# nelpy/ghost

Hardware: AMD Instinct MI355X
Metric: Msamples/s CWT (128ch x 1e6 samp x 100 scales); % HBM roofline; 1/2/4/8 GPU (higher is better)
Workload: dtype f32

## Files before the change

ghost_amd/csrc/api.cpp:

```cpp
#include <hip/hip_runtime.h>

#include <algorithm>
#include <cmath>
#include <cstdio>
#include <cstdlib>
#include <cstring>
#include <exception>
#include <map>
#include <new>
#include <string>
#include <vector>

#include "../../include/ghostcwt.h"
#include "../../include/ghostcwt_debug.h"
#include <memory>

#include "errors.h"
#include "host_out.h"
#include "interp.h"
#include "kernels.h"
#include "morse_exact.h"
#include "morlet_exact.h"
#include "options.h"
#include "planner.h"

using namespace gcwt;

namespace {

thread_local std::string g_err;


int set_err(int code, const std::string& msg) {
  g_err = msg;
  return code;
}

int hip_err(hipError_t e, const char* what) {
  g_err = std::string(what) + ": " + hipGetErrorString(e);
  return e == hipErrorOutOfMemory ? GCWT_ERR_NOMEM : GCWT_ERR_HIP;
}

#define HIP_TRY(call)                                  \
  do {                                                 \
    hipError_t e_ = (call);                            \
    if (e_ != hipSuccess) return hip_err(e_, #call);   \
  } while (0)

struct EpochDev {
  SynthItemDev* items = nullptr;
  int n_items = 0;
  SynthLevelDev* levels = nullptr;
  Synth7Item* items7 = nullptr;
  Synth7Level* levels7 = nullptr;
  int n_items7 = 0;
  Synth7Item* items7w = nullptr;
  int n_items7w = 0;
  Synth7Item* items7n = nullptr;
  int n_items7n = 0;
  SynthiItem* items_i = nullptr;
  SynthiLevel* levels_i = nullptr;
  int n_items_i = 0;
  SynthpItem* items_p[2] = {nullptr, nullptr};
  SynthpLevel* levels_p = nullptr;
  int n_items_p[2] = {0, 0};
  PredLevel* pred_levels = nullptr;
};

constexpr int64_t kFullbandCacheBytes = (int64_t)16 << 30;

enum Stage { ST_MEAN = 0, ST_FWD, ST_DECIM, ST_BLOCK, ST_SYNTH, ST_DIRECT, ST_FULLBAND, ST_INTERP, ST_BLOCKCONV, ST_COUNT };

}

struct gcwt_plan {
  HostPlan hp;
  bool uploaded = false;
  int profiling = 0;
  int synth_cols = 32;
  int synth7_narrow_r = 2;
  bool fuse_blocks = true;
  int synth_kernel = 7;
  bool prune_inputs = true;
  bool fast_fft = true;
  int drop_stores = 0;
  bool clock_probe = false;
  bool use_synth16 = false;
  int device = -1;
  hipStream_t stream = nullptr;
  hipStream_t aux[2] = {nullptr, nullptr};
  bool level_streams = true;
  bool use_synthp = false;
  bool use_graphs = true;
  bool fullband4 = true;
  int fullband_group = 0;
  int64_t fullband_cache_cap = 0;
  bool hfull_cache_full = false;
  int synth7_order = 0;
  int synthp_help = -1;
  int synthp_lgnb = -1;
  int interp_lgnb = -1;
  int interp_grid = -1;
  bool last_fold = false;
  bool fold_mean = true;
  bool synth_streams = false;
  hipStream_t cur = nullptr;
  bool high_precision = true;
  double2* d_y = nullptr;
  int64_t y_stride = 0;
  double2* d_tw64 = nullptr;
  float2* d_x = nullptr;
  float2* d_xr = nullptr;
  float2* d_xb = nullptr;
  float2* d_bank = nullptr;
  float* d_gain = nullptr;
  float* d_gain_lv = nullptr;
  float2* d_half_tw = nullptr;
  float2* d_psi = nullptr;
  float2* d_psi_tail = nullptr;
  float2* d_psi_lit = nullptr;
  unsigned long long* d_probe = nullptr;
  double* d_amps = nullptr;
  float2* d_xs = nullptr;
  int64_t xs_stride = 0;
  float2* d_z = nullptr;
  int64_t z_half = 0;
  int z_sets = 1;
  float2* d_hfull = nullptr;
  std::map<std::pair<int, int>, float2*> hfull_cache;
  int64_t hfull_cache_bytes = 0;
  float2* d_tw4096 = nullptr;
  float2* d_tw256 = nullptr;
  float2* d_level_tw = nullptr;
  double* d_sums = nullptr;
  int32_t* d_scale_list = nullptr;
  int n_listed = 0;
  int32_t* d_scale_aux = nullptr;
  float* d_interp_coef = nullptr;
  BankScale* d_bank_sc = nullptr;
  DirectScale* d_direct_sc = nullptr;
  float2* d_bc_h = nullptr;
  int32_t* d_bc_rows = nullptr;
  float2* d_bc_x = nullptr;
  float2* d_bc_tw = nullptr;
  std::vector<EpochDev> ep_dev;
  int64_t max_direct_len = 0;
  float* d_in = nullptr;
  size_t d_in_bytes = 0;
  void* d_out = nullptr;
  size_t d_out_bytes = 0;
  HostOut host_out;
  std::vector<hipEvent_t> ev_pool;
  size_t ev_used = 0;
  struct Span { int stage; hipEvent_t a, b; };
  std::vector<Span> spans;
  gcwt_timings last{};
  bool have_timings = false;
  bool have_means = false;
  bool detect = false;
  float* d_hist = nullptr;
  float* d_bands = nullptr;
  float* d_pred = nullptr;
  hipStream_t det_stream = nullptr;
  int32_t* d_scale_level = nullptr;
  int32_t* d_scale_length = nullptr;
  std::vector<float> last_pred;
  float* h_pred = nullptr;
  float last_worst = 0.f;
  int last_rerouted = 0;
  float auto_threshold = 1.5e-6f;
  float kappa_eps = 1.6e-7f;
  float oob_tol = 2.5e-8f;
  int last_batch_slots = 0;
  int last_batch = 0, last_rows = 0;
  double last_pt = 0;
  gcwt_plan* sub_plan[2] = {nullptr, nullptr};
  bool is_sub_plan = false;
  const unsigned char* run_mask = nullptr;
  unsigned char* d_run_mask = nullptr;
  struct GraphKey {
    const void* x = nullptr; const void* out = nullptr;
    int64_t r0 = 0, r1 = 0, row_len = 0; bool reuse = false;
    bool operator==(const GraphKey& o) const {
      return x == o.x && out == o.out && r0 == o.r0 && r1 == o.r1 && row_len == o.row_len && reuse == o.reuse;
    }
  };
  GraphKey graph_key, graph_seen;
  hipGraphExec_t graph_exec = nullptr;
// ... 122 lines not shown
int gcwt_device_pci_bus_id(int device, char* buf, size_t buflen) {
  if (!buf || buflen < 16) return set_err(GCWT_ERR_INVALID, "buffer of at least 16 bytes needed");
  HIP_TRY(hipDeviceGetPCIBusId(buf, (int)buflen, device));
  return GCWT_OK;
}

int gcwt_set_device(int device) {
  int n = 0;
  if (hipGetDeviceCount(&n) != hipSuccess || n == 0) {
    (void)hipGetLastError();
    return set_err(GCWT_ERR_NO_DEVICE, "no HIP device: libghostcwt needs an AMD GPU (gfx950); there is no CPU path");
  }
  if (device < 0 || device >= n) return set_err(GCWT_ERR_NO_DEVICE, "no such device (gcwt_device_count tells how many there are)");
  HIP_TRY(hipSetDevice(device));
  return GCWT_OK;
}
int gcwt_current_device(int* device) {
  if (!device) return set_err(GCWT_ERR_INVALID, "NULL argument");
  HIP_TRY(hipGetDevice(device));
  return GCWT_OK;
}

int gcwt_device_memory(size_t* free_bytes, size_t* total_bytes) {
  if (!free_bytes || !total_bytes) return set_err(GCWT_ERR_INVALID, "NULL argument");
  HIP_TRY(hipMemGetInfo(free_bytes, total_bytes));
  return GCWT_OK;
}
int gcwt_device_malloc(void** ptr, size_t bytes) { HIP_TRY(hipMalloc(ptr, bytes ? bytes : 1)); return GCWT_OK; }
int gcwt_device_free(void* ptr) { HIP_TRY(hipFree(ptr)); return GCWT_OK; }
int gcwt_memcpy_h2d(void* dst, const void* src, size_t bytes) {
  HIP_TRY(hipMemcpy(dst, src, bytes, hipMemcpyHostToDevice)); return GCWT_OK;
}
int gcwt_memcpy_d2h(void* dst, const void* src, size_t bytes) {
  HIP_TRY(hipMemcpy(dst, src, bytes, hipMemcpyDeviceToHost)); return GCWT_OK;
}
int gcwt_device_memset(void* dst, int value, size_t bytes) {
  HIP_TRY(hipMemset(dst, value, bytes)); return GCWT_OK;
}
int gcwt_device_synchronize(void) { HIP_TRY(hipDeviceSynchronize()); return GCWT_OK; }
int gcwt_host_alloc(void** ptr, size_t bytes) {
  if (!ptr) return set_err(GCWT_ERR_INVALID, "NULL argument");
  HIP_TRY(hipHostMalloc(ptr, bytes ? bytes : 1, hipHostMallocDefault));
  return GCWT_OK;
}
int gcwt_host_free(void* ptr) { HIP_TRY(hipHostFree(ptr)); return GCWT_OK; }
int gcwt_rows_to_host(const float* d_src, int64_t src_pitch, int64_t n_rows, int64_t row_elems, void* dst,
                      int64_t dst_pitch, int flags) {
  return guarded([&] {
    if (!d_src || !dst) return set_err(GCWT_ERR_INVALID, "NULL argument");
    if (n_rows < 0 || row_elems < 0 || src_pitch < row_elems || dst_pitch < row_elems)
      return set_err(GCWT_ERR_INVALID, "bad rectangle (rows, elements per row, pitches)");
    if (!(flags & GCWT_HOST_PINNED) && dst_pitch != row_elems)
      return set_err(GCWT_ERR_INVALID, "a destination that is not page-locked takes dense rows (dst_pitch = row_elems)");
    HIP_TRY(rows_to_host(d_src, src_pitch, n_rows, row_elems, dst, dst_pitch, (flags & GCWT_OUT_F64) != 0,
                         (flags & GCWT_HOST_PINNED) != 0));
    return (int)GCWT_OK;
  });
}

static int gcwt_plan_create_impl(gcwt_plan** out, const gcwt_params* params) {
  if (!out || !params) return set_err(GCWT_ERR_INVALID, "NULL argument");
  *out = nullptr;
  std::unique_ptr<gcwt_plan> owner(new (std::nothrow) gcwt_plan());
  gcwt_plan* p = owner.get();
  if (!p) return set_err(GCWT_ERR_NOMEM, "out of host memory");
  std::string err;
  int rc = build_host_plan(*params, &p->hp, &err);
  if (rc != GCWT_OK) return set_err(rc, err);
  p->hp.prm.freqs_hz = p->hp.freqs.data();
  p->hp.prm.epoch_bounds = p->hp.bounds.data();
  p->hp.prm.n_epochs = (int32_t)(p->hp.bounds.size() / 2);
  p->device = params->device;
  p->high_precision = p->hp.high_precision;
  p->use_synth16 = option_or("synth16", 0) == 1;
  p->synth_cols = option_or("synth_cols", 32) == 16 ? 16 : 32;
  p->synth7_narrow_r = (int)option_or("synth7_narrow_r", 2);
  p->fuse_blocks = option_or("fuse_blocks", 1) != 0;
  p->prune_inputs = option_or("prune_inputs", 1) != 0;
  p->fast_fft = option_or("slow_fft", 0) == 0;
  p->level_streams = option_or("level_streams", 1) != 0;
  if (option_is_set("interp_grid")) p->interp_grid = option_or("interp_grid", 0) != 0;
  p->synth_streams = option_or("synth_streams", 0) != 0;
  p->fold_mean = option_or("fold_mean", 1) != 0;
  p->interp_lgnb = (int)option_or("interp_lgnb", -1);
  p->use_synthp = kMeasureBuild && option_or("synthp", 0) != 0;
  p->synthp_lgnb = (int)option_or("synthp_lgnb", -1);
  p->synthp_help = (int)option_or("synthp_help", -1);
  p->use_graphs = option_or("graphs", 1) != 0;
  p->synth7_order = (int)option_or("synth7_order", 0);
  p->auto_threshold = 1e-9f * (float)option_or("auto_threshold_ppb", 1500);
  p->kappa_eps = 1e-9f * (float)option_or("auto_kappa_ppb", 160);
  p->oob_tol = 1e-12f * (float)option_or("auto_oob_ppt", 25000);
  p->fullband_group = (int)option_or("fullband_group", 0);
  p->fullband4 = option_or("fullband4", 1) != 0;
  p->synth_kernel = kMeasureBuild && option_or("synth_kernel", 7) == 8 ? 8 : 7;
  p->drop_stores = kMeasureBuild && option_is_set("synth_drop_stores") ? (int)std::max<long long>(1, option_or("synth_drop_stores", 1)) : 0;
  p->clock_probe = kMeasureBuild && option_is_set("clock_probe");
  for (const auto& s : p->hp.scales)
    if (s.method == GCWT_SCALE_DIRECT) p->max_direct_len = std::max(p->max_direct_len, s.length);
  *out = owner.release();
  return GCWT_OK;
}

void gcwt_plan_destroy(gcwt_plan* plan) {
  if (!plan) return;
  if (plan->uploaded || plan->stream) {
    if (plan->device >= 0) (void)hipSetDevice(plan->device);
    free_dev(plan);
  }
  delete plan;
}

int gcwt_plan_get_info(const gcwt_plan* plan, gcwt_plan_info* info) {
  if (!plan || !info) return set_err(GCWT_ERR_INVALID, "NULL argument");
  const HostPlan& hp = plan->hp;
  info->abi_version = GCWT_ABI_VERSION;
  info->n_levels = (int32_t)hp.levels.size();
  info->n_direct = hp.n_direct;
  info->n_spectral = (int32_t)hp.scales.size() - hp.n_direct - hp.n_fullband - hp.n_blockconv;
  info->n_fullband = hp.n_fullband;
  info->n_blockconv = hp.n_blockconv;
  info->reserved = 0;
  info->n_interp = 0;
  for (const auto& l : hp.levels)
    if (level_kernel(plan, l) == LK_INTERP) info->n_interp += (int32_t)l.scales.size();
  info->block = hp.block;
  int r = 1;
  for (const auto& l : hp.levels) r = std::max(r, l.decimation);
  info->max_decimation = r;
  info->fft_length = hp.max_p;
  {
    const int64_t C = hp.prm.n_channels, slots = C * hp.max_batch;
    int64_t extra = 0, xs = 0, y = 0;
    for (const EpochPlan& ep : hp.epochs) {
      for (size_t l = 0; l < hp.levels.size(); ++l)
        if (hp.levels[l].band_shift > 0) xs = std::max<int64_t>(xs, ep.lv[l].m);
      const int rows = ep.p1 >= 4 && hp.n_fullband == 0 ? ep.p1 / 2 + 1 : ep.p1;
      y = std::max<int64_t>(y, (int64_t)rows * kRowLen);
    }
    extra += 8 * 3 * slots * xs;
    if (hp.high_precision && plan->fast_fft && hp.n_direct + hp.n_blockconv < hp.prm.n_freqs)
      extra += 16 * (slots * y + 8192);
    extra += 8 * (2 * (int64_t)hp.direct_total + (int64_t)hp.n_direct);
    int64_t listed = 0;
    for (const LevelPlan& lp : hp.levels) listed += (int64_t)lp.scales.size();
    extra += 4 * (listed + 8) * 256 + 8 * 256 * (int64_t)hp.levels.size();
    extra += 8 * (int64_t)channel_sum_doubles((size_t)C) + 4 * (int64_t)hp.interp_coef.size();
    if (hp.high_precision && !hp.exact_only) {
      int64_t max_rows = 1;
      for (const EpochPlan& ep : hp.epochs) max_rows = std::max<int64_t>(max_rows, ep.p1);
      extra += 4 * (slots * (max_rows * kRowBands + kSpecBands) + (int64_t)hp.prm.n_freqs * (int64_t)hp.epochs.size());
    }
    if (hp.n_fullband > 0)
      extra += std::min<int64_t>(plan->uploaded ? plan->fullband_cache_cap : kFullbandCacheBytes,
                                 8 * (int64_t)hp.n_fullband * hp.max_p * (int64_t)hp.epochs.size());
    info->workspace_bytes = hp.workspace_bytes + extra;
    for (const gcwt_plan* sub : plan->sub_plan) {
      gcwt_plan_info si{};
      if (sub && gcwt_plan_get_info(sub, &si) == GCWT_OK) info->workspace_bytes += si.workspace_bytes;
    }
  }
  info->out_bytes = (int64_t)hp.out_elem_bytes * hp.prm.n_channels * hp.prm.n_freqs *
                    stride_cols(0, hp.prm.n_samples, plan->out_stride);
  return GCWT_OK;
}

// ... 246 lines not shown
    if (p->synth7_order == 1) std::reverse(items7.begin(), items7.end());
    else if (p->synth7_order == 2) {
      std::vector<std::vector<Synth7Item>> by(hp.levels.size());
      for (const auto& it : items7) by[(size_t)it.level].push_back(it);
      std::vector<Synth7Item> mixed;
      std::vector<double> pos(by.size(), 0.0);
      size_t left = items7.size();
      while (left) {
        size_t best = by.size(); double frac = 2.0;
        for (size_t l = 0; l < by.size(); ++l)
          if (pos[l] < (double)by[l].size() && pos[l] / (double)by[l].size() < frac) { frac = pos[l] / (double)by[l].size(); best = l; }
        mixed.push_back(by[best][(size_t)pos[best]]);
        pos[best] += 1.0; --left;
      }
      items7.swap(mixed);
    }
    p->ep_dev[e].n_items7 = (int)items7.size();
    p->ep_dev[e].n_items7w = (int)items7w.size();
    p->ep_dev[e].n_items7n = (int)items7n.size();
    if ((rc = upload_vec(&p->ep_dev[e].items7n, items7n, p->stream))) return bail(rc);
    if ((rc = upload_vec(&p->ep_dev[e].items7, items7, p->stream))) return bail(rc);
    if ((rc = upload_vec(&p->ep_dev[e].items7w, items7w, p->stream))) return bail(rc);
    if ((rc = upload_vec(&p->ep_dev[e].levels7, lv7, p->stream))) return bail(rc);
    std::vector<SynthiItem> items_i;
    std::vector<std::pair<int, int>> pending;
    std::vector<SynthiLevel> lvi(hp.levels.size());
    std::vector<int> order;
    std::vector<int> order_p;
    for (size_t l = 0; l < hp.levels.size(); ++l)
      if (level_kernel(p, hp.levels[l]) == LK_INTERP)
        (level_pipelined(p, hp.levels[l]) ? order_p : order).push_back((int)l);
    std::sort(order.begin(), order.end(),
              [&](int x, int y) { return hp.levels[x].decimation > hp.levels[y].decimation; });
    std::sort(order_p.begin(), order_p.end(),
              [&](int x, int y) { return hp.levels[x].decimation > hp.levels[y].decimation; });
    for (int l : order) {
      const LevelPlan& lp = hp.levels[l];
      int lgq = 0;
      while ((1 << lgq) < lp.interp_q) ++lgq;
      int lgnb = lp.decimation <= 32 && lp.interp_q <= 2 ? 1 : 0;
      if (p->interp_lgnb >= 0) lgnb = std::min(p->interp_lgnb, 2);
      while (lgnb > 0 && (lp.interp_q << lgnb) > kInterpMaxPhases) --lgnb;
      if (lp.interp_q < 2 || lp.interp_q > kInterpMaxPhases || (lp.interp_q & (lp.interp_q - 1)) ||
          lp.interp_factor * lp.interp_q != lp.decimation || lp.interp_factor < 4 ||
          lp.interp_factor > kInterpMaxFactor || lp.scales.size() > 256 || lp.halo < 16 ||
          lp.hop != hp.block - 2 * lp.halo || lp.hop < 1 || hp.block != 256 || (lp.interp_taps != 6 && lp.interp_taps != 8))
        return bail(set_err(GCWT_ERR_INVALID, "internal: interpolated level outside the kernel's limits"));
      lvi[l] = {lp.decimation, lp.interp_q, lgq, lp.interp_factor, lp.hop, lp.halo, ep.lv[l].nblk,
                (int32_t)lp.scales.size(), scale_off[l], ep.lv[l].blk_lo, lgnb, lp.interp_taps, lp.twiddle_offset,
                ep.lv[l].xr_offset, ep.lv[l].m - 1, lp.coef_offset};
      pending.push_back({l, lgnb});
    }
    {
      const int64_t n_ch_slots = (int64_t)hp.prm.n_channels * std::max(1, ep.batch_count);
      int64_t target = (int64_t)2 << 20;
      std::vector<int64_t> item_bytes;
      for (int attempt = 0;; ++attempt) {
        items_i.clear();
        item_bytes.clear();
        for (const auto& pl : pending) {
          const LevelPlan& lp = hp.levels[pl.first];
          const int nb = 1 << pl.second, ns = kInterpCols / (lp.interp_q * nb);
          const int n_pass = ((int)lp.scales.size() + ns - 1) / ns;
          const int64_t pass_bytes = (int64_t)ns * nb * lp.hop * lp.decimation * 4;
          const int run = (int)std::max<int64_t>(1, std::min<int64_t>(n_pass, target / std::max<int64_t>(1, pass_bytes)));
          const int wps = (lp.hop * (lp.decimation >> 2) + 63) >> 6;
          const int quads = (wps + 3) / 4;
          const int parts = run > 1 ? 1 : (int)std::min<int64_t>(quads, (pass_bytes + target - 1) / target);
          for (int b0 = 0; b0 < ep.lv[pl.first].nblk; b0 += nb)
            for (int p0 = 0; p0 < n_pass; p0 += run)
              for (int part = 0; part < parts; ++part) {
                const int lo = 4 * (int)((int64_t)quads * part / parts);
                const int hi = std::min(wps, 4 * (int)((int64_t)quads * (part + 1) / parts));
                const int np = std::min(run, n_pass - p0);
                items_i.push_back({(int32_t)pl.first, b0, p0, np, lo, hi});
                item_bytes.push_back((int64_t)np * pass_bytes * (hi - lo) / std::max(1, wps));
              }
        }
        if ((int64_t)items_i.size() * n_ch_slots >= 3072 || target <= ((int64_t)1 << 19) || attempt > 6) break;
        target >>= 1;
      }
      std::vector<size_t> order(items_i.size());
      for (size_t i = 0; i < order.size(); ++i) order[i] = i;
      std::stable_sort(order.begin(), order.end(), [&](size_t x, size_t y) { return item_bytes[x] > item_bytes[y]; });
      std::vector<SynthiItem> sorted(items_i.size());
      for (size_t i = 0; i < order.size(); ++i) sorted[i] = items_i[order[i]];
      items_i.swap(sorted);
    }
    p->ep_dev[e].n_items_i = (int)items_i.size();
    if ((rc = upload_vec(&p->ep_dev[e].items_i, items_i, p->stream))) return bail(rc);
    if ((rc = upload_vec(&p->ep_dev[e].levels_i, lvi, p->stream))) return bail(rc);
    {
      std::vector<SynthpLevel> lvp(hp.levels.size());
      std::vector<SynthpItem> items_p[2];
      std::vector<int64_t> bytes_p[2];
      const int64_t n_ch_slots = (int64_t)hp.prm.n_channels * std::max(1, ep.batch_count);
      for (int l : order_p) {
        const LevelPlan& lp = hp.levels[l];
        int lgnb = lp.decimation <= 16 ? 2 : lp.decimation <= 32 ? 1 : 0;
        if (p->synthp_lgnb >= 0) lgnb = std::min(p->synthp_lgnb, 2);
        if (lp.interp_factor * 2 != lp.decimation || lp.halo < 16 || lp.hop != hp.block - 2 * lp.halo || lp.hop < 1 ||
            hp.block != 256 || (lp.hop * lp.decimation) % (4 * lp.interp_factor) != 0)
          return bail(set_err(GCWT_ERR_INVALID, "internal: pipelined level outside the kernel's limits"));
        const double tasks = 4.0 * lp.hop * lp.decimation / 256.0;
        int help = (int)std::lround(128.0 * std::max(0.0, (tasks - 27.0) / (4.0 * tasks)));
        if (p->synthp_help >= 0) help = std::min(p->synthp_help, 64);
        lvp[l] = {lp.decimation, lp.interp_factor, lp.hop, lp.halo, ep.lv[l].nblk, (int32_t)lp.scales.size(),
                  scale_off[l], ep.lv[l].blk_lo, lgnb, n_plain[l], (int32_t)(l * 256), help, lp.twiddle_offset,
                  ep.lv[l].xr_offset, ep.lv[l].m - 1, lp.coef_offset};
      }
      int64_t target = (int64_t)2 << 20;
      for (int attempt = 0;; ++attempt) {
        for (int k = 0; k < 2; ++k) { items_p[k].clear(); bytes_p[k].clear(); }
        for (int l : order_p) {
          const LevelPlan& lp = hp.levels[l];
          const int nb = 1 << lvp[l].log2nb, ns = kSynthpSlots / nb;
          const int n_rounds = ((int)lp.scales.size() + ns - 1) / ns;
          const int64_t round_bytes = (int64_t)ns * nb * lp.hop * lp.decimation * 4;
          const int run = (int)std::max<int64_t>(1, std::min<int64_t>(n_rounds, target / std::max<int64_t>(1, round_bytes)));
          const int k = lp.interp_factor == 4 ? 1 : 0;
          for (int b0 = 0; b0 < ep.lv[l].nblk; b0 += nb)
            for (int r0 = 0; r0 < n_rounds; r0 += run) {
              const int nr = std::min(run, n_rounds - r0);
              items_p[k].push_back({(int32_t)l, b0, r0, nr});
              bytes_p[k].push_back((int64_t)nr * round_bytes);
            }
        }
        if ((int64_t)(items_p[0].size() + items_p[1].size()) * n_ch_slots >= 2048 || target <= ((int64_t)1 << 19) || attempt > 6) break;
        target >>= 1;
      }
      for (int k = 0; k < 2; ++k) {
        std::vector<size_t> ord(items_p[k].size());
        for (size_t i = 0; i < ord.size(); ++i) ord[i] = i;
        std::stable_sort(ord.begin(), ord.end(), [&](size_t x, size_t y) { return bytes_p[k][x] > bytes_p[k][y]; });
        std::vector<SynthpItem> sorted(items_p[k].size());
        for (size_t i = 0; i < ord.size(); ++i) sorted[i] = items_p[k][ord[i]];
        p->ep_dev[e].n_items_p[k] = (int)sorted.size();
        if ((rc = upload_vec(&p->ep_dev[e].items_p[k], sorted, p->stream))) return bail(rc);
      }
      if ((rc = upload_vec(&p->ep_dev[e].levels_p, lvp, p->stream))) return bail(rc);
    }
  }

  {
    bool long_mode = false, any_level = false;
    for (const EpochPlan& ep : hp.epochs) long_mode = long_mode || ep.long_a > 1;
    std::vector<int32_t> scale_level((size_t)S, -1);
    for (int i = 0; i < S; ++i)
      if (hp.scales[i].method == GCWT_SCALE_SPECTRAL && hp.scales[i].level >= 0) { scale_level[(size_t)i] = hp.scales[i].level; any_level = true; }
    p->detect = hp.high_precision && !hp.exact_only && p->d_y && !long_mode && any_level;
    if (p->detect) {
      const int64_t slots = (int64_t)C * hp.max_batch;
      int64_t max_rows = 1;
      for (const EpochPlan& ep : hp.epochs)
        max_rows = std::max<int64_t>(max_rows, ep.p1);
      if ((rc = dev_alloc(&p->d_hist, (size_t)(slots * max_rows * kRowBands)))) return bail(rc);
      if ((rc = dev_alloc(&p->d_bands, (size_t)(slots * kSpecBands)))) return bail(rc);
      if ((rc = dev_alloc(&p->d_pred, (size_t)S * (size_t)C * hp.epochs.size()))) return bail(rc);
      if ((rc = upload_vec(&p->d_scale_level, scale_level, p->stream))) return bail(rc);
      std::vector<int32_t> scale_length((size_t)S);
      for (int i = 0; i < S; ++i) scale_length[(size_t)i] = (int32_t)std::min<int64_t>(hp.scales[i].length, (int64_t)1 << 30);
      if ((rc = upload_vec(&p->d_scale_length, scale_length, p->stream))) return bail(rc);
      for (size_t e = 0; e < hp.epochs.size(); ++e) {
        const EpochPlan& ep = hp.epochs[e];
        if (ep.batch_count == 0) continue;
        std::vector<PredLevel> pl(hp.levels.size());
        for (size_t l = 0; l < hp.levels.size(); ++l) {
          const LevelPlan& lp = hp.levels[l];
          const LevelPlan& own = hp.levels[lp.xr_owner >= 0 ? (size_t)lp.xr_owner : l];
          pl[l] = {lp.scales.empty() ? 0 : lp.decimation, lp.band_shift, 0.f, 0.f};
// ... 94 lines not shown
    } else {
      for (const auto& g : gaps) {
        he = launch_zero_range(dout, row_len * elem, (int64_t)C * S, stride_cols(r0, g.first, K) * elem,
                               stride_cols(g.first, g.second, K) * elem, st);
        if (he != hipSuccess) return hip_err(he, "zero_range");
      }
    }
  }

  bool any_fft = hp.n_direct + hp.n_blockconv < S;
  if (hmask) {
    any_fft = false;
    for (int i = 0; i < S; ++i)
      any_fft = any_fft || (hmask[i] && hp.scales[i].method != GCWT_SCALE_DIRECT && hp.scales[i].method != GCWT_SCALE_BLOCKCONV);
  }
  const bool fast_fft = p->fast_fft;
  for (size_t e0 = 0; any_fft && e0 < hp.epochs.size();) {
    const EpochPlan& ep = hp.epochs[e0];
    const size_t count = (size_t)std::max(1, ep.batch_count);
    SegIn sin{};
    SegOut sout{};
    PredSegs psegs{};
    int nb = 0;
    for (size_t i = 0; i < count; ++i) {
      const EpochPlan& m = hp.epochs[e0 + i];
      const int64_t w_lo = std::max(m.core0, r0) - m.start, w_hi = std::min(m.core1, r1) - m.start;
      if (w_hi <= w_lo) continue;
      psegs.seg[nb] = (int32_t)(e0 + i);
      sin.x_off[nb] = m.start;
      sin.n_valid[nb] = m.ne;
      sin.n_lead[nb] = m.lead;
      sin.ramp_lo[nb] = m.ramp_lo;
      sin.ramp_hi[nb] = m.ramp_hi;
      sout.seg_col[nb] = m.start - r0;
      sout.w_lo[nb] = w_lo;
      sout.w_hi[nb] = w_hi;
      ++nb;
    }
    e0 += count;
    if (nb == 0) continue;
    sin.n_channels = sout.n_channels = psegs.n_channels = C;
    sout.os = os;
    const int slots = C * nb;
    const int64_t P = ep.p_store, Pt = ep.p;
    const int P1 = ep.p1, A = ep.long_a;
    const bool hermitian = fast_fft && P1 >= 4 && hp.n_fullband == 0;
    const int rows_a = hermitian ? P1 / 2 + 1 : P1;
    if (p->d_y) {
      for (int a = 0; a < A; ++a) {
        RUN(ST_FWD, launch_fwd64_cols(dx, p->d_y, P1, N, p->y_stride, P, p->d_tw64, p->d_sums, inv_n, sin, nb,
                                      rows_a, st, A, a, fold));
        if (fold) RUN(ST_MEAN, launch_channel_sum_final(p->d_sums, C, fold_parts(P1), st));
        RUN(ST_FWD, launch_fwd64_rows(p->d_y, p->d_x, rows_a, p->y_stride, P, p->d_tw64, slots,
                                      hp.n_fullband > 0 ? kRowLen : kRowLen / 2, hermitian ? P1 : 0, st, a, A, Pt,
                                      p->detect ? p->d_hist : nullptr, P1, fold ? p->d_sums : nullptr, inv_n, ep.ne, P1));
      }
      if (p->detect) {
        hipEvent_t bands_done;
        int rc_ = get_event(p, &bands_done);
        if (rc_) return rc_;
        he = hipEventRecord(bands_done, st);
        if (he == hipSuccess) he = hipStreamWaitEvent(p->det_stream, bands_done, 0);
        if (he != hipSuccess) return hip_err(he, "detector fork");
        he = launch_band_sums(p->d_hist, P1, p->d_bands, slots, p->det_stream);
        if (he != hipSuccess) return hip_err(he, "launch_band_sums");
        he = launch_precision_predict(p->d_bands, p->d_gain, p->d_scale_level, p->d_scale_length, p->ep_dev[ep.batch_first].pred_levels, S,
                                      (int)hp.levels.size(), (double)Pt, p->kappa_eps, p->oob_tol, p->d_pred, nullptr, nullptr, slots, psegs,
                                      p->det_stream);
        if (he != hipSuccess) return hip_err(he, "launch_precision_predict");
        p->last_batch_slots = slots; p->last_batch = ep.batch_first; p->last_pt = (double)Pt; p->last_rows = P1;
      }
    } else if (A > 1) {
      return set_err(GCWT_ERR_UNSUPPORTED, "internal: long mode without the float64 forward transform");
    } else {
    RUN(ST_FWD, launch_fft_cols_batch(dx, p->d_x, P1, kRowLen, N, P, P1 > 1 ? P : 0, p->d_tw4096,
                                      fast_fft ? p->d_tw256 : nullptr, p->d_sums, inv_n, sin, nb, st,
                                      rows_a));
    RUN(ST_FWD, launch_fft_rows(-1, p->d_x, p->d_x, kRowLen, rows_a, kRowLen, kRowLen, P, P, 0,
                                p->d_tw4096, fast_fft ? p->d_tw256 : nullptr, 1.0f, slots, st,
                                hp.n_fullband > 0 ? kRowLen : kRowLen / 2, hermitian ? P1 : 0));
    }
    const bool fused_blocks = p->fuse_blocks && p->synth_kernel == 7 && !p->use_synth16;
    const bool side = p->level_streams && hp.levels.size() > 2;
    std::vector<int> stream_of(hp.levels.size(), 0);
    if (side) {
      double load[3] = {0.0, 0.0, 0.0};
      std::vector<size_t> order;
      for (size_t l = 0; l < hp.levels.size(); ++l)
        if (hp.levels[l].xr_owner == (int)l) order.push_back(l);
      std::stable_sort(order.begin(), order.end(), [&](size_t a, size_t b) { return ep.lv[a].m > ep.lv[b].m; });
      for (size_t l : order) {
        const int k = (int)(std::min_element(load, load + 3) - load);
        stream_of[l] = k;
        load[k] += 40e-6 + 32.0 * (double)ep.lv[l].m * (double)slots / 4.5e12;
      }
      for (size_t l = 0; l < hp.levels.size(); ++l) stream_of[l] = stream_of[hp.levels[l].xr_owner];
    }
    bool forked[2] = {false, false};
    hipEvent_t spectrum_ready = nullptr;
    if (side) {
      int rc_ = get_event(p, &spectrum_ready);
      if (rc_) return rc_;
      he = hipEventRecord(spectrum_ready, st);
      if (he != hipSuccess) return hip_err(he, "hipEventRecord");
    }
    for (size_t l = 0; l < hp.levels.size(); ++l) {
      const LevelPlan& lp = hp.levels[l];
      const EpochLevel& el = ep.lv[l];
      float2* xr = p->d_xr + el.xr_offset;
      hipStream_t ls = st;
      RowTaper taper;
      if (p->high_precision && lp.taper_hi > 0.0 && lp.band_shift == 0) {
        const double k1 = lp.taper_hi * (double)Pt / (2.0 * M_PI), k0 = 0.5 * k1;
        if (k1 - k0 >= 1.0) { taper.p1 = P1; taper.k0 = (float)k0; taper.inv_width = (float)(1.0 / (k1 - k0)); }
      }
      if (side) {
        const int k = stream_of[l];
        ls = k == 0 ? st : p->aux[k - 1];
        if (k > 0 && !forked[k - 1]) {
          he = hipStreamWaitEvent(ls, spectrum_ready, 0);
          if (he != hipSuccess) return hip_err(he, "hipStreamWaitEvent");
          forked[k - 1] = true;
        }
        p->cur = ls;
      }
      if (lp.xr_owner != (int)l) {
      } else if (lp.decimation / A <= kMaxTwoPassDecimation) {
        const int Q = kRowLen * A / lp.decimation;
        const float2* src = p->d_x;
        int64_t src_row = kRowLen, src_cstride = P;
        if (lp.band_shift > 0) {
          const int64_t U = (int64_t)lp.band_shift * el.m / hp.block;
          if (U % P1 != 0 || U / P1 > Q) return set_err(GCWT_ERR_INVALID, "internal: band shift does not slice the spectrum");
          float2* xs = p->d_xs + (int64_t)stream_of[l] * slots * p->xs_stride;
          RUN(ST_DECIM, launch_shift_gather(p->d_x, xs, P1, Q, (int)(U / P1), kRowLen, P, p->xs_stride, slots, ls));
          src = xs; src_row = Q; src_cstride = p->xs_stride;
        }
        RUN(ST_DECIM, launch_fft_rows(+1, src, xr, Q, P1, src_row, Q, src_cstride, hp.max_xr,
                                      P1 > 1 ? el.m : 0, p->d_tw4096,
                                      fast_fft ? p->d_tw256 : nullptr, 1.0f, slots, ls, 0, 0, taper));
        if (P1 > 1)
          RUN(ST_DECIM, launch_fft_cols(+1, false, xr, xr, P1, Q, hp.max_xr, hp.max_xr, 0,
                                        p->d_tw4096, fast_fft ? p->d_tw256 : nullptr, p->d_sums,
                                        inv_n, 0, slots, ls));
      } else {
        const int n1 = (int)std::min<int64_t>(P1, el.m);
        const int q = (int)(el.m / n1);
        RUN(ST_DECIM, launch_level_small(p->d_x, xr, n1, q, kRowLen, P, hp.max_xr, p->d_tw4096, slots, ls, taper));
      }
      const float scale = (float)(1.0 / ((double)hp.block * (double)Pt));
      const LevelKernel lk = level_kernel(p, lp);
      if (lk == LK_SYNTH16 || (lk == LK_SYNTH7 && !fused_blocks))
        RUN(ST_BLOCK, launch_block_fft(xr, p->d_xb + el.xb_offset, el.m, lp.hop, lp.halo, el.blk_lo,
                                       el.nblk, hp.max_xr, hp.max_xb, p->d_tw256, scale, slots, ls));
    }
    if (side) {
      p->cur = nullptr;
      for (int k = 0; k < 2; ++k) {
        if (!forked[k]) continue;
        hipEvent_t done;
        int rc_ = get_event(p, &done);
        if (rc_) return rc_;
        he = hipEventRecord(done, p->aux[k]);
        if (he == hipSuccess) he = hipStreamWaitEvent(st, done, 0);
        if (he != hipSuccess) return hip_err(he, "level streams join");
      }
    }
    const EpochDev& dev = p->ep_dev[ep.batch_first];
    hipStream_t si = st;
    if (dev.n_items_i > 0) {
      const bool beside = p->synth_streams && (dev.n_items7 > 0 || dev.n_items7w > 0 || dev.n_items7n > 0 || dev.n_items > 0);
      if (beside) {
        hipEvent_t levels_done;
        int rc_ = get_event(p, &levels_done);
        if (rc_) return rc_;
        he = hipEventRecord(levels_done, st);
        if (he == hipSuccess) he = hipStreamWaitEvent(p->aux[0], levels_done, 0);
        if (he != hipSuccess) return hip_err(he, "synthesis fork");
        si = p->aux[0];
      }
      SynthiArgs ai{};
      ai.tw256 = p->d_tw256;
      ai.level_tw = p->d_level_tw;
      ai.items = dev.items_i;
      ai.levels = dev.levels_i;
      ai.scale_list = p->d_scale_list;
      ai.scale_aux = p->d_scale_aux;
      ai.gain = p->d_gain;
      ai.coef = p->d_interp_coef;
      ai.out = dout;
      ai.row_len = row_len;
      ai.xr = p->d_xr;
      ai.xr_cstride = hp.max_xr;
      ai.xb_scale = (float)(1.0 / ((double)hp.block * (double)Pt));
      ai.n_scales = S;
      ai.channels_fastest = p->interp_grid >= 0 ? p->interp_grid : (slots <= 32 ? 1 : 0);
      if (dev.n_items_i > 65535) ai.channels_fastest = 0;
      ai.seg = sout;
      p->cur = si;
      if (strided) RUN(ST_INTERP, launch_synthis(mode, ai, dev.n_items_i, slots, si));
      else RUN(ST_INTERP, launch_synthi(mode, ai, dev.n_items_i, slots, si));
      p->cur = nullptr;
    }
    for (int k = 0; k < 2; ++k) {
      if (dev.n_items_p[k] == 0) continue;
      SynthpArgs ap{};
      ap.tw256 = p->d_tw256;
      ap.level_tw = p->d_level_tw;
      ap.items = dev.items_p[k];
      ap.levels = dev.levels_p;
      ap.scale_list = p->d_scale_list;
      ap.scale_aux = p->d_scale_aux;
      ap.gain_lv = p->d_gain_lv;
      ap.level_half_tw = p->d_half_tw;
      ap.coef = p->d_interp_coef;
      ap.out = dout;
      ap.row_len = row_len;
      ap.xr = p->d_xr;
      ap.xr_cstride = hp.max_xr;
      ap.xb_scale = (float)(1.0 / ((double)hp.block * (double)Pt));
      ap.n_scales = S;
      ap.channels_fastest = p->interp_grid >= 0 ? p->interp_grid : (slots <= 32 ? 1 : 0);
      if (dev.n_items_p[k] > 65535) ap.channels_fastest = 0;
      ap.flags = 0;
      ap.seg = sout;
      p->cur = si;
#ifdef GCWT_MEASURE
      if (strided) return set_err(GCWT_ERR_UNSUPPORTED, "output stride with the pipelined interpolating kernel");
      RUN(ST_INTERP, launch_synthp(mode, ap, dev.n_items_p[k], slots, k == 1, si));
#else
      return set_err(GCWT_ERR_INVALID, "internal: a level planned for the measure build's pipelined kernel");
#endif
      p->cur = nullptr;
    }
    if (dev.n_items > 0) {
      SynthArgs a{};
      a.xb = p->d_xb;
      a.bank = p->d_bank;
      a.tw256 = p->d_tw256;
      a.level_tw = p->d_level_tw;
      a.items = dev.items;
      a.levels = dev.levels;
      a.out = dout;
      a.xb_cstride = hp.max_xb;
      a.row_len = row_len;
      a.n_scales = S;
      a.seg = sout;
      RUN(ST_SYNTH, launch_synth(mode, a, dev.n_items, slots, st));
    }
    for (int variant = 0; variant < 3; ++variant) {
      const int wide = variant == 2;
      const int cols7 = variant == 0 ? 16 : p->synth_cols;
      const int n7 = variant == 0 ? dev.n_items7n : wide ? dev.n_items7w : dev.n_items7;
      if (n7 == 0) continue;
      Synth7Args a7{};
      a7.xb = p->d_xb;
      a7.bank = p->d_bank;
      a7.tw256 = p->d_tw256;
      a7.level_tw = p->d_level_tw;
      a7.items = variant == 0 ? dev.items7n : wide ? dev.items7w : dev.items7;
      a7.levels = dev.levels7;
      a7.scale_list = p->d_scale_list;
      a7.gain = p->d_gain;
      a7.gain_lv = p->d_gain_lv;
      a7.level_half_tw = p->d_half_tw;
      a7.complex_gains = hp.morlet ? 1 : 0;
      a7.out = dout;
      a7.xb_cstride = hp.max_xb;
      a7.row_len = row_len;
      a7.n_scales = S;
      a7.drop_stores = p->drop_stores;
      a7.seg = sout;
      a7.clock_probe = p->d_probe;
      if (fused_blocks) {
        a7.xr = p->d_xr;
        a7.xr_cstride = hp.max_xr;
        a7.xb_scale = (float)(1.0 / ((double)hp.block * (double)Pt));
      }
      if (strided) {
        RUN(ST_SYNTH, launch_synth7s(mode, cols7, a7, n7, slots, st));
        continue;
      }
#ifdef GCWT_MEASURE
      if (p->synth_kernel == 8 && variant == 1)
        RUN(ST_SYNTH, launch_synth8(mode, p->synth_cols, a7, n7, slots, st));
      else
#endif
        RUN(ST_SYNTH, launch_synth7(mode, cols7, wide != 0, a7, n7, slots, st));
    }
    if (si != st) {
      hipEvent_t interp_done;
      int rc_ = get_event(p, &interp_done);
      if (rc_) return rc_;
      he = hipEventRecord(interp_done, si);
      if (he == hipSuccess) he = hipStreamWaitEvent(st, interp_done, 0);
      if (he != hipSuccess) return hip_err(he, "synthesis join");
    }
    if (p->detect && p->d_y) {
      hipEvent_t pred_done;
      int rc_ = get_event(p, &pred_done);
      if (rc_) return rc_;
      he = hipEventRecord(pred_done, p->det_stream);
      if (he == hipSuccess) he = hipStreamWaitEvent(st, pred_done, 0);
      if (he != hipSuccess) return hip_err(he, "detector join");
    }
    if (p->profiling && !hp.levels.empty()) p->last.synth_launches++;
    auto response = [&](int i, int scratch, const float2** h_out) -> int {
      const auto cached = p->hfull_cache.find({i, P1});
      if (cached != p->hfull_cache.end()) { *h_out = cached->second; return GCWT_OK; }
      float2* dst = p->d_hfull + (int64_t)scratch * hp.max_p;
      float2* keep = nullptr;
      const int64_t bytes = (int64_t)sizeof(float2) * P;
      if (!p->hfull_cache_full && p->hfull_cache_bytes + bytes <= p->fullband_cache_cap) {
        if (hipMalloc((void**)&keep, (size_t)bytes) == hipSuccess) dst = keep;
        else {
          (void)hipGetLastError();
// ... 685 lines not shown
```

ghost_amd/csrc/options.cpp:

```cpp
#include "options.h"

#include <cctype>
#include <cstdlib>
#include <cstring>
#include <map>
#include <mutex>
#include <string>

#include "kernels.h"

namespace gcwt {
namespace {

const char* const kSelect[] = {"synth16", "synth_cols", "fuse_blocks", "slow_fft", "level_streams", "interp_grid",
                               "synth_streams", "interp_lgnb", "merge_levels", "split_levels", "interp",
                               "batch_bytes", "stage_floats", "fullband_group", "blockconv",
                               "direct_max_len", "graphs", "plan_threads", "fullband_cache_mb", "auto_threshold_ppb", "auto_kappa_ppb", "auto_oob_ppt", "synth7_order", "host_widen", "host_threads", "fullband4", "cu_count", "synth7_narrow_r", "fold_mean"};
const char* const kMeasureOnly[] = {"halo_margin", "interp_q", "interp_taps", "interp_min_r", "prune_inputs", "clock_phases",
                                    "synth_kernel", "synth_drop_stores", "clock_probe", "synthi_pad_kb",
                                    "synthp", "synthp_lgnb", "synthp_help"};
const char* const kEnvBudgets[] = {"batch_bytes", "stage_floats"};

std::mutex g_mu;
std::map<std::string, long long>& table() {
  static std::map<std::string, long long> t;
  return t;
}

template <size_t N>
bool in_list(const char* name, const char* const (&list)[N]) {
  for (const char* s : list)
    if (!strcmp(s, name)) return true;
  return false;
}

bool from_env(const char* name, long long* v) {
  std::string var = "GHOSTCWT_";
  for (const char* c = name; *c; ++c) var.push_back((char)toupper((unsigned char)*c));
  const char* e = getenv(var.c_str());
  if (!e) return false;
  *v = *e ? atoll(e) : 1;
  return true;
}

bool lookup(const char* name, long long* v) {
  {
    std::lock_guard<std::mutex> lock(g_mu);
    auto it = table().find(name);
    if (it != table().end()) { *v = it->second; return true; }
  }
  if (kMeasureBuild || in_list(name, kEnvBudgets)) return from_env(name, v);
  return false;
}

}

long long option_or(const char* name, long long dflt) {
  long long v;
  return lookup(name, &v) ? v : dflt;
}

bool option_is_set(const char* name) {
  long long v;
  return lookup(name, &v);
}

int option_set(const char* name, long long value, bool clear) {
  if (!name) return -1;
  const bool measure_only = in_list(name, kMeasureOnly);
  if (!measure_only && !in_list(name, kSelect)) return -1;
  if (measure_only && !kMeasureBuild) return -2;
  std::lock_guard<std::mutex> lock(g_mu);
  if (clear) table().erase(name);
  else table()[name] = value;
  return 0;
}

}
```

Baseline: 9592.

## Split interpolating synthesis launch by decimation and optionally overlap it with level streams

Interpolating synthesis work items are now sorted so that levels below a decimation threshold come first, and the kernel is launched as two separate parts at that boundary. An opt-in early_interp mode keeps the interpolating levels on the main stream, processes them first, and delays joining the side level streams until after the interpolating kernels, so interpolation can overlap the other levels' FFT work. The default path now always issues the split launch, which adds a second kernel launch and changes work-item order. Early scheduling stays off by default.

Result: faster. 9700, median of 6 (+1.1%).

```diff
diff --git a/ghost_amd/csrc/api.cpp b/ghost_amd/csrc/api.cpp
--- a/ghost_amd/csrc/api.cpp
+++ b/ghost_amd/csrc/api.cpp
@@ -61,6 +61,7 @@
   SynthiItem* items_i = nullptr;
   SynthiLevel* levels_i = nullptr;
   int n_items_i = 0;
+  int split_i = 0;
   SynthpItem* items_p[2] = {nullptr, nullptr};
   SynthpLevel* levels_p = nullptr;
   int n_items_p[2] = {0, 0};
@@ -104,6 +105,8 @@
   bool last_fold = false;
   bool fold_mean = true;
   bool synth_streams = false;
+  int interp_split_r = 64;
+  bool early_interp = false;
   hipStream_t cur = nullptr;
   bool high_precision = true;
   double2* d_y = nullptr;
@@ -392,6 +395,8 @@
   if (option_is_set("interp_grid")) p->interp_grid = option_or("interp_grid", 0) != 0;
   p->synth_streams = option_or("synth_streams", 0) != 0;
   p->fold_mean = option_or("fold_mean", 1) != 0;
+  p->early_interp = option_or("early_interp", 0) != 0;
+  p->interp_split_r = (int)std::min<long long>(1 << 30, std::max<long long>(0, option_or("interp_split_r", 64)));
   p->interp_lgnb = (int)option_or("interp_lgnb", -1);
   p->use_synthp = kMeasureBuild && option_or("synthp", 0) != 0;
   p->synthp_lgnb = (int)option_or("synthp_lgnb", -1);
@@ -804,10 +809,16 @@
       }
       std::vector<size_t> order(items_i.size());
       for (size_t i = 0; i < order.size(); ++i) order[i] = i;
-      std::stable_sort(order.begin(), order.end(), [&](size_t x, size_t y) { return item_bytes[x] > item_bytes[y]; });
+      const int split_r = p->interp_split_r;
+      std::vector<char> late(items_i.size());
+      for (size_t i = 0; i < late.size(); ++i) late[i] = hp.levels[(size_t)items_i[i].level].decimation >= split_r;
+      std::stable_sort(order.begin(), order.end(), [&](size_t x, size_t y) {
+        return late[x] != late[y] ? late[x] < late[y] : item_bytes[x] > item_bytes[y];
+      });
       std::vector<SynthiItem> sorted(items_i.size());
       for (size_t i = 0; i < order.size(); ++i) sorted[i] = items_i[order[i]];
       items_i.swap(sorted);
+      p->ep_dev[e].split_i = (int)std::count(late.begin(), late.end(), (char)0);
     }
     p->ep_dev[e].n_items_i = (int)items_i.size();
     if ((rc = upload_vec(&p->ep_dev[e].items_i, items_i, p->stream))) return bail(rc);
@@ -1068,15 +1079,28 @@
     }
     const bool fused_blocks = p->fuse_blocks && p->synth_kernel == 7 && !p->use_synth16;
     const bool side = p->level_streams && hp.levels.size() > 2;
+    const EpochDev& dev = p->ep_dev[ep.batch_first];
+    std::vector<char> in_h(hp.levels.size(), 0);
+    bool any_h = false;
+    for (size_t l = 0; l < hp.levels.size(); ++l)
+      if (level_kernel(p, hp.levels[l]) == LK_INTERP) {
+        in_h[hp.levels[l].xr_owner >= 0 ? (size_t)hp.levels[l].xr_owner : l] = 1;
+        any_h = true;
+      }
+    for (size_t l = 0; l < hp.levels.size(); ++l)
+      if (hp.levels[l].xr_owner >= 0) in_h[l] = in_h[(size_t)hp.levels[l].xr_owner];
+    const bool early = side && p->early_interp && p->profiling != 1 && !p->synth_streams && any_h &&
+                       dev.n_items_i + dev.n_items_p[0] + dev.n_items_p[1] > 0;
     std::vector<int> stream_of(hp.levels.size(), 0);
     if (side) {
       double load[3] = {0.0, 0.0, 0.0};
       std::vector<size_t> order;
       for (size_t l = 0; l < hp.levels.size(); ++l)
-        if (hp.levels[l].xr_owner == (int)l) order.push_back(l);
+        if (hp.levels[l].xr_owner == (int)l && !(early && in_h[l])) order.push_back(l);
       std::stable_sort(order.begin(), order.end(), [&](size_t a, size_t b) { return ep.lv[a].m > ep.lv[b].m; });
+      const int k0 = early ? 1 : 0;
       for (size_t l : order) {
-        const int k = (int)(std::min_element(load, load + 3) - load);
+        const int k = (int)(std::min_element(load + k0, load + 3) - load);
         stream_of[l] = k;
         load[k] += 40e-6 + 32.0 * (double)ep.lv[l].m * (double)slots / 4.5e12;
       }
@@ -1090,7 +1114,9 @@
       he = hipEventRecord(spectrum_ready, st);
       if (he != hipSuccess) return hip_err(he, "hipEventRecord");
     }
-    for (size_t l = 0; l < hp.levels.size(); ++l) {
+    for (size_t li = 0; li < (early ? 2 : 1) * hp.levels.size(); ++li) {
+      const size_t l = li % hp.levels.size();
+      if (early && (in_h[l] != 0) != (li < hp.levels.size())) continue;
       const LevelPlan& lp = hp.levels[l];
       const EpochLevel& el = ep.lv[l];
       float2* xr = p->d_xr + el.xr_offset;
@@ -1140,10 +1166,11 @@
         RUN(ST_BLOCK, launch_block_fft(xr, p->d_xb + el.xb_offset, el.m, lp.hop, lp.halo, el.blk_lo,
                                        el.nblk, hp.max_xr, hp.max_xb, p->d_tw256, scale, slots, ls));
     }
-    if (side) {
-      p->cur = nullptr;
+    if (side) p->cur = nullptr;
+    auto join_levels = [&]() -> int {
       for (int k = 0; k < 2; ++k) {
         if (!forked[k]) continue;
+        forked[k] = false;
         hipEvent_t done;
         int rc_ = get_event(p, &done);
         if (rc_) return rc_;
@@ -1151,8 +1178,12 @@
         if (he == hipSuccess) he = hipStreamWaitEvent(st, done, 0);
         if (he != hipSuccess) return hip_err(he, "level streams join");
       }
-    }
-    const EpochDev& dev = p->ep_dev[ep.batch_first];
+      return GCWT_OK;
+    };
+    if (!early) {
+      int rc_ = join_levels();
+      if (rc_) return rc_;
+    }
     hipStream_t si = st;
     if (dev.n_items_i > 0) {
       const bool beside = p->synth_streams && (dev.n_items7 > 0 || dev.n_items7w > 0 || dev.n_items7n > 0 || dev.n_items > 0);
@@ -1184,8 +1215,13 @@
       if (dev.n_items_i > 65535) ai.channels_fastest = 0;
       ai.seg = sout;
       p->cur = si;
-      if (strided) RUN(ST_INTERP, launch_synthis(mode, ai, dev.n_items_i, slots, si));
-      else RUN(ST_INTERP, launch_synthi(mode, ai, dev.n_items_i, slots, si));
+      for (int part = 0; part < 2; ++part) {
+        const int first = part == 0 ? 0 : dev.split_i, n_part = part == 0 ? dev.split_i : dev.n_items_i - dev.split_i;
+        if (n_part == 0) continue;
+        ai.items = dev.items_i + first;
+        if (strided) RUN(ST_INTERP, launch_synthis(mode, ai, n_part, slots, si));
+        else RUN(ST_INTERP, launch_synthi(mode, ai, n_part, slots, si));
+      }
       p->cur = nullptr;
     }
     for (int k = 0; k < 2; ++k) {
@@ -1218,6 +1254,10 @@
       return set_err(GCWT_ERR_INVALID, "internal: a level planned for the measure build's pipelined kernel");
 #endif
       p->cur = nullptr;
+    }
+    if (early) {
+      int rc_ = join_levels();
+      if (rc_) return rc_;
     }
     if (dev.n_items > 0) {
       SynthArgs a{};
diff --git a/ghost_amd/csrc/options.cpp b/ghost_amd/csrc/options.cpp
--- a/ghost_amd/csrc/options.cpp
+++ b/ghost_amd/csrc/options.cpp
@@ -15,7 +15,8 @@
 const char* const kSelect[] = {"synth16", "synth_cols", "fuse_blocks", "slow_fft", "level_streams", "interp_grid",
                                "synth_streams", "interp_lgnb", "merge_levels", "split_levels", "interp",
                                "batch_bytes", "stage_floats", "fullband_group", "blockconv",
-                               "direct_max_len", "graphs", "plan_threads", "fullband_cache_mb", "auto_threshold_ppb", "auto_kappa_ppb", "auto_oob_ppt", "synth7_order", "host_widen", "host_threads", "fullband4", "cu_count", "synth7_narrow_r", "fold_mean"};
+                               "direct_max_len", "graphs", "plan_threads", "fullband_cache_mb", "auto_threshold_ppb", "auto_kappa_ppb", "auto_oob_ppt", "synth7_order", "host_widen", "host_threads", "fullband4", "cu_count", "synth7_narrow_r", "fold_mean",
+                               "early_interp", "interp_split_r"};
 const char* const kMeasureOnly[] = {"halo_margin", "interp_q", "interp_taps", "interp_min_r", "prune_inputs", "clock_phases",
                                     "synth_kernel", "synth_drop_stores", "clock_probe", "synthi_pad_kb",
                                     "synthp", "synthp_lgnb", "synthp_help"};
```
